# jnvance/DMRG.x

Hardware: AMD Instinct MI355X
Metric: superblock MatMults/sec inside the ground-state eigensolve (Lanczos step = 1 MatMult + reorthogonalisation) (higher is better)
Workload: dtype f64

## Files before the change

dmrg.x_amd/csrc/eigs.hip:

```cpp
#include "krylov.h"
#include <mutex>
#include <algorithm>
#include <chrono>
#include <cmath>
#include <cstring>
#include <cstddef>

namespace dmrgx {
namespace {

constexpr int DOT_BLOCKS = 1024, DOT_THREADS = 256, DOT_CHUNK = 8, MAX_NCV = 64, FUSE_NV = 24, GD_NV = 8;

template <bool VEC2>
__global__ void __launch_bounds__(DOT_THREADS)
multi_dot_kernel(const double* __restrict__ V, int64_t ldv, int nv, const double* __restrict__ w, int64_t n, double* __restrict__ partial)
{
    __shared__ double red[DOT_THREADS / 64][DOT_CHUNK];
    const int v0 = blockIdx.y * DOT_CHUNK;
    double acc[DOT_CHUNK];
#pragma unroll
    for (int i = 0; i < DOT_CHUNK; ++i) acc[i] = 0.0;
    if (VEC2) {
        const double2* __restrict__ w2 = reinterpret_cast<const double2*>(w);
        for (int64_t e = (int64_t)blockIdx.x * DOT_THREADS + threadIdx.x; e < n / 2; e += (int64_t)gridDim.x * DOT_THREADS) {
            const double2 wv = w2[e];
#pragma unroll
            for (int i = 0; i < DOT_CHUNK; ++i) {
                const int v = v0 + i;
                if (v < nv) { const double2 x = reinterpret_cast<const double2*>(V + (int64_t)v * ldv)[e]; acc[i] += x.x * wv.x + x.y * wv.y; }
                else if (v == nv) acc[i] += wv.x * wv.x + wv.y * wv.y;
            }
        }
    } else {
        for (int64_t e = (int64_t)blockIdx.x * DOT_THREADS + threadIdx.x; e < n; e += (int64_t)gridDim.x * DOT_THREADS) {
            const double wv = w[e];
#pragma unroll
            for (int i = 0; i < DOT_CHUNK; ++i) {
                const int v = v0 + i;
                if (v < nv) acc[i] += V[(int64_t)v * ldv + e] * wv;
                else if (v == nv) acc[i] += wv * wv;
            }
        }
    }
    const int lane = threadIdx.x & 63, wave = threadIdx.x >> 6;
#pragma unroll
    for (int i = 0; i < DOT_CHUNK; ++i) {
        const double s = wave_sum(acc[i]);
        if (lane == 0) red[wave][i] = s;
    }
    __syncthreads();
    if (threadIdx.x < DOT_CHUNK) {
        double s = 0.0;
        for (int wv = 0; wv < DOT_THREADS / 64; ++wv) s += red[wv][threadIdx.x];
        partial[(int64_t)(v0 + threadIdx.x) * gridDim.x + blockIdx.x] = s;
    }
}

__global__ void __launch_bounds__(DOT_THREADS)
reduce_partials_kernel(const double* __restrict__ partial, double* __restrict__ out, int count, int nblk)
{
    const int i = blockIdx.x;
    if (i >= count) return;
    const double s = sum_partials<DOT_THREADS>(partial + (int64_t)i * nblk, nblk);
    if (threadIdx.x == 0) out[i] = s;
}

__global__ void __launch_bounds__(DOT_THREADS)
multi_axpy_kernel(const double* __restrict__ V, int64_t ldv, int nv, const double* __restrict__ c, double* __restrict__ w, int64_t n,
                  double* __restrict__ partial, double* __restrict__ hacc)
{
    __shared__ double cs[MAX_NCV + 1];
    if (threadIdx.x < nv) cs[threadIdx.x] = c[threadIdx.x];
    __syncthreads();
    if (blockIdx.x == 0 && threadIdx.x < nv && hacc) hacc[threadIdx.x] += cs[threadIdx.x];
    double nrm = 0.0;
    for (int64_t e = (int64_t)blockIdx.x * DOT_THREADS + threadIdx.x; e < n; e += (int64_t)gridDim.x * DOT_THREADS) {
        double x = w[e];
        for (int i = 0; i < nv; ++i) x -= cs[i] * V[(int64_t)i * ldv + e];
        w[e] = x;
        nrm += x * x;
    }
    nrm = block_sum<DOT_THREADS>(nrm);
    if (threadIdx.x == 0) partial[blockIdx.x] = nrm;
}

template <int NVMAX>
__global__ void __launch_bounds__(DOT_THREADS)
axpy_dot_kernel(const double* __restrict__ V, int64_t ldv, int nv, const double* __restrict__ c, double* __restrict__ w, int64_t n,
                double* __restrict__ partial, double* __restrict__ hacc)
{
    __shared__ double cs[NVMAX];
    __shared__ double red[DOT_THREADS / 64][NVMAX + 1];
    if (threadIdx.x < nv) cs[threadIdx.x] = c[threadIdx.x];
    __syncthreads();
    if (blockIdx.x == 0 && threadIdx.x < nv && hacc) hacc[threadIdx.x] += cs[threadIdx.x];
    double acc[NVMAX + 1];
#pragma unroll
    for (int i = 0; i <= NVMAX; ++i) acc[i] = 0.0;
    for (int64_t e = (int64_t)blockIdx.x * DOT_THREADS + threadIdx.x; e < n; e += (int64_t)gridDim.x * DOT_THREADS) {
        double v[NVMAX];
#pragma unroll
        for (int i = 0; i < NVMAX; ++i) v[i] = i < nv ? V[(int64_t)i * ldv + e] : 0.0;
        double x = w[e];
#pragma unroll
        for (int i = 0; i < NVMAX; ++i) if (i < nv) x -= cs[i] * v[i];
        w[e] = x;
#pragma unroll
        for (int i = 0; i < NVMAX; ++i) if (i < nv) acc[i] += v[i] * x;
        acc[NVMAX] += x * x;
    }
    const int lane = threadIdx.x & 63, wave = threadIdx.x >> 6;
#pragma unroll
    for (int i = 0; i <= NVMAX; ++i) {
        if (i < nv || i == NVMAX) {
            const double s2 = wave_sum(acc[i]);
            if (lane == 0) red[wave][i] = s2;
        }
    }
    __syncthreads();
    if (threadIdx.x <= nv) {
        const int src = threadIdx.x < nv ? threadIdx.x : NVMAX;
        double s2 = 0.0;
        for (int wv = 0; wv < DOT_THREADS / 64; ++wv) s2 += red[wv][src];
        partial[(int64_t)threadIdx.x * gridDim.x + blockIdx.x] = s2;
    }
}

template <bool VEC2>
__global__ void __launch_bounds__(DOT_THREADS)
axpy_normalise_kernel(const double* __restrict__ V, int64_t ldv, int nv, const double* __restrict__ c, const double* __restrict__ w,
                      double* __restrict__ dst, int64_t n, double* __restrict__ beta2_out, double* __restrict__ hacc)
{
    __shared__ double cs[MAX_NCV + 2];
    if (threadIdx.x <= nv) cs[threadIdx.x] = c[threadIdx.x];
    __syncthreads();
    if (blockIdx.x == 0 && threadIdx.x < nv && hacc) hacc[threadIdx.x] += cs[threadIdx.x];
    double s2 = cs[nv], sc = 0.0;
    for (int i = 0; i < nv; ++i) { s2 -= cs[i] * cs[i]; sc += cs[i] * cs[i]; }
    s2 = s2 > 0.0 ? s2 : 0.0;
    if (blockIdx.x == 0 && threadIdx.x == 0 && beta2_out) *beta2_out = s2;
    const double inv = s2 > 1e-290 ? 1.0 / sqrt(s2) : 0.0;
    if (sc <= 1e-27 * cs[nv]) nv = 0;
    if (VEC2) {
        const double2* __restrict__ w2 = reinterpret_cast<const double2*>(w);
        double2* __restrict__ d2 = reinterpret_cast<double2*>(dst);
        for (int64_t e = (int64_t)blockIdx.x * DOT_THREADS + threadIdx.x; e < n / 2; e += (int64_t)gridDim.x * DOT_THREADS) {
            double2 x = w2[e];
            for (int i = 0; i < nv; ++i) { const double2 v = reinterpret_cast<const double2*>(V + (int64_t)i * ldv)[e]; x.x -= cs[i] * v.x; x.y -= cs[i] * v.y; }
            x.x *= inv; x.y *= inv;
            d2[e] = x;
        }
    } else {
        for (int64_t e = (int64_t)blockIdx.x * DOT_THREADS + threadIdx.x; e < n; e += (int64_t)gridDim.x * DOT_THREADS) {
            double x = w[e];
            for (int i = 0; i < nv; ++i) x -= cs[i] * V[(int64_t)i * ldv + e];
            dst[e] = x * inv;
        }
    }
}

__global__ void norm_after_projection_kernel(const double* __restrict__ c, int nv, double* __restrict__ nrm2)
{
    if (threadIdx.x == 0 && blockIdx.x == 0) { double s = c[nv]; for (int i = 0; i < nv; ++i) s -= c[i] * c[i]; *nrm2 = s > 0.0 ? s : 0.0; }
}

__global__ void scale_copy_kernel(const double* __restrict__ src, double* __restrict__ dst, int64_t n, const double* __restrict__ nrm2)
{
    const double s2 = *nrm2;
    const double inv = s2 > 1e-290 ? 1.0 / sqrt(s2) : 0.0;
    for (int64_t e = (int64_t)blockIdx.x * blockDim.x + threadIdx.x; e < n; e += (int64_t)gridDim.x * blockDim.x) dst[e] = src[e] * inv;
}

__global__ void __launch_bounds__(DOT_THREADS)
basis_rotate_kernel(const double* __restrict__ V, int64_t ldv, int m, const double* __restrict__ Q, int ldq, int k,
                    double* __restrict__ out, int64_t ldo, int64_t n)
{
    __shared__ double qs[MAX_NCV * DOT_CHUNK];
    const int j0 = blockIdx.y * DOT_CHUNK;
    for (int t = threadIdx.x; t < m * DOT_CHUNK; t += DOT_THREADS) {
        const int i = t / DOT_CHUNK, j = t % DOT_CHUNK;
        qs[t] = (j0 + j < k) ? Q[i * ldq + j0 + j] : 0.0;
    }
    __syncthreads();
    for (int64_t e = (int64_t)blockIdx.x * DOT_THREADS + threadIdx.x; e < n; e += (int64_t)gridDim.x * DOT_THREADS) {
        double acc[DOT_CHUNK];
#pragma unroll
        for (int j = 0; j < DOT_CHUNK; ++j) acc[j] = 0.0;
        for (int i = 0; i < m; ++i) {
            const double v = V[(int64_t)i * ldv + e];
#pragma unroll
            for (int j = 0; j < DOT_CHUNK; ++j) acc[j] += v * qs[i * DOT_CHUNK + j];
        }
#pragma unroll
        for (int j = 0; j < DOT_CHUNK; ++j) if (j0 + j < k) out[(int64_t)(j0 + j) * ldo + e] = acc[j];
    }
}

constexpr int GD_MAX = FUSE_NV;
constexpr int GD_LD = GD_MAX;
struct GdState {
    double G[GD_MAX * GD_LD];
    double Y[GD_MAX * GD_LD];
    double th[GD_MAX];
    double y[GD_MAX];
    double yprev[GD_MAX];
    double Q[GD_MAX * GD_LD];
    double theta;
    double hv0_2;
    double e0[GD_MAX];
    int after_restart;
    int pad_;
};

constexpr int RITZ_THREADS = 64;
__global__ void __launch_bounds__(RITZ_THREADS)
gd_ritz_kernel(GdState* __restrict__ S, const double* __restrict__ col_src, int col_is_partial, int nblk, int mm, int warm, int restart, int keep)
{
    __shared__ double A[GD_MAX][GD_MAX + 1], Qa[GD_MAX][GD_MAX + 1], Yn[GD_MAX][GD_MAX + 1], Yp[GD_MAX][GD_MAX + 1];
    __shared__ double col[GD_MAX + 1], cs_c[GD_MAX / 2], cs_s[GD_MAX / 2], dg[GD_MAX], thp[GD_MAX], ths[GD_MAX];
    __shared__ int pp[GD_MAX / 2], qq[GD_MAX / 2], perm[GD_MAX];
    __shared__ double offn, dgn;
    const int tid = threadIdx.x, lane = tid;
    const int j = mm - 1;
    if (warm && mm > 1) {
        for (int e = tid; e < (mm - 1) * (mm - 1); e += RITZ_THREADS) Yp[e / (mm - 1)][e % (mm - 1)] = S->Y[(e / (mm - 1)) * GD_LD + e % (mm - 1)];
        if (tid < mm - 1) thp[tid] = S->th[tid];
    }
    const double yold = tid < GD_MAX ? S->y[tid] : 0.0;
    const int was_restart = S->after_restart;
    if (col_is_partial) {
        constexpr int PER = DOT_BLOCKS / RITZ_THREADS;
        for (int i0 = 0; i0 <= mm; i0 += 4) {
            double t[4][PER];
#pragma unroll
            for (int g = 0; g < 4; ++g)
#pragma unroll
                for (int u = 0; u < PER; ++u) t[g][u] = (i0 + g <= mm && tid + u * RITZ_THREADS < nblk) ? col_src[(int64_t)(i0 + g) * nblk + tid + u * RITZ_THREADS] : 0.0;
#pragma unroll
            for (int g = 0; g < 4; ++g) {
                double v = 0.0;
#pragma unroll
                for (int u = 0; u < PER; ++u) v += t[g][u];
                v = wave_sum(v);
                if (lane == 0 && i0 + g <= mm) col[i0 + g] = v;
            }
        }
    } else if (tid <= mm) col[tid] = col_src[tid];
    __syncthreads();
    if (tid < mm) { S->G[tid * GD_LD + j] = col[tid]; S->G[j * GD_LD + tid] = col[tid]; }
    if (tid == 0 && mm == 1) S->hv0_2 = col[1];
    if (tid < GD_MAX && mm == 1) S->e0[tid] = tid == 0 ? 1.0 : 0.0;
    if (tid < mm) S->yprev[tid] = was_restart ? (tid == 0 ? 1.0 : 0.0) : (tid < mm - 1 ? yold : 0.0);
    if (tid == 0) S->after_restart = restart;
    const int n = (mm + 1) & ~1;
    const int mp = mm - 1;
    for (int e = tid; e < n * n; e += RITZ_THREADS) {
        const int a = e / n, b = e % n;
        double v = 0.0;
        if (a < mm && b < mm) {
            if (!warm || mp == 0) v = (a == j || b == j) ? col[a == j ? b : a] : S->G[a * GD_LD + b];
            else if (a < mp && b < mp) v = a == b ? thp[a] : 0.0;
            else if (a == mp && b == mp) v = col[j];
            else {
                const int i = a == mp ? b : a;
                for (int k = 0; k < mp; ++k) v += Yp[k][i] * col[k];
            }
        }
        A[a][b] = v;
        Qa[a][b] = a == b ? 1.0 : 0.0;
    }
    __syncthreads();
    constexpr int UMAX = (GD_MAX / 2 * GD_MAX + RITZ_THREADS - 1) / RITZ_THREADS;
    int wk[UMAX], wi[UMAX];
#pragma unroll
    for (int u = 0; u < UMAX; ++u) { const int e = tid + u * RITZ_THREADS; wk[u] = e < (n / 2) * n ? e / n : -1; wi[u] = e % n; }
    for (int sweep = 0; sweep < 30 && n > 1; ++sweep) {
        {
            double off = 0.0, dgs = 0.0;
#pragma unroll
            for (int u = 0; u < UMAX; ++u) {
                if (wk[u] < 0) continue;
                const double v0 = A[wk[u]][wi[u]], v1 = A[wk[u] + n / 2][wi[u]];
                if (wk[u] == wi[u]) dgs += v0 * v0; else off += v0 * v0;
                if (wk[u] + n / 2 == wi[u]) dgs += v1 * v1; else off += v1 * v1;
            }
            off = wave_sum(off); dgs = wave_sum(dgs);
            if (lane == 0) { offn = off; dgn = dgs; }
        }
        __syncthreads();
        if (offn <= 1e-29 * (dgn + offn) || offn == 0.0) break;
        for (int r = 0; r < n - 1; ++r) {
            if (tid < n / 2) {
                const int k = tid;
                int p0 = r + k, q0 = r - k + (n - 1);
                if (p0 >= n - 1) p0 -= n - 1;
                if (q0 >= n - 1) q0 -= n - 1;
                if (k == 0) { p0 = r; q0 = n - 1; }
                const int p = min(p0, q0), q = max(p0, q0);
                const double apq = A[p][q];
                double c = 1.0, sn = 0.0;
                if (apq != 0.0) {
                    const double th = 0.5 * (A[q][q] - A[p][p]);
                    const double h = sqrt(th * th + apq * apq);
                    const double t = apq / (th + (th >= 0.0 ? h : -h));
                    c = rsqrt(1.0 + t * t); sn = t * c;
                }
                pp[k] = p; qq[k] = q; cs_c[k] = c; cs_s[k] = sn;
            }
            __syncthreads();
#pragma unroll
            for (int u = 0; u < UMAX; ++u) {
                if (wk[u] < 0) continue;
                const int k = wk[u], i = wi[u];
                const int p = pp[k], q = qq[k];
                const double c = cs_c[k], sn = cs_s[k];
                const double aip = A[i][p], aiq = A[i][q];
                A[i][p] = c * aip - sn * aiq; A[i][q] = sn * aip + c * aiq;
                const double qip = Qa[i][p], qiq = Qa[i][q];
                Qa[i][p] = c * qip - sn * qiq; Qa[i][q] = sn * qip + c * qiq;
            }
            __syncthreads();
#pragma unroll
            for (int u = 0; u < UMAX; ++u) {
                if (wk[u] < 0) continue;
                const int k = wk[u], i = wi[u];
                const int p = pp[k], q = qq[k];
                const double c = cs_c[k], sn = cs_s[k];
                const double api = A[p][i], aqi = A[q][i];
                A[p][i] = i == q ? 0.0 : c * api - sn * aqi; A[q][i] = i == p ? 0.0 : sn * api + c * aqi;
            }
            __syncthreads();
        }
    }
    if (tid < mm) dg[tid] = A[tid][tid];
    __syncthreads();
    if (tid < mm) {
        int rank = 0;
        for (int o = 0; o < mm; ++o) rank += (dg[o] < dg[tid] || (dg[o] == dg[tid] && o < tid)) ? 1 : 0;
        perm[rank] = tid;
    }
    __syncthreads();
    for (int e = tid; e < mm * mm; e += RITZ_THREADS) {
        const int i = e / mm, cidx = e % mm;
        const int src = perm[cidx];
        double v;
        if (!warm || mp == 0 || i == mp) v = Qa[i][src];
        else { v = 0.0; for (int k = 0; k < mp; ++k) v += Yp[i][k] * Qa[k][src]; }
        Yn[i][cidx] = v;
    }
    __syncthreads();
    for (int e = tid; e < mm * mm; e += RITZ_THREADS) S->Y[(e / mm) * GD_LD + (e % mm)] = Yn[e / mm][e % mm];
    if (tid < mm) { ths[tid] = dg[perm[tid]]; S->th[tid] = ths[tid]; S->y[tid] = Yn[tid][0]; }
    if (tid == 0) S->theta = dg[perm[0]];
    if (!restart) return;
    __syncthreads();
    const int kk = keep + 1;
    {
        double pv = lane < mm ? S->yprev[lane] : 0.0;
        for (int pass = 0; pass < 2; ++pass)
            for (int c = 0; c < keep; ++c) {
                const double qc = lane < mm ? Yn[lane][c] : 0.0;
                double d = qc * pv;
#pragma unroll
                for (int o = 32; o > 0; o >>= 1) d += __shfl_xor(d, o, 64);
                pv -= d * qc;
            }
        double nn = pv * pv;
#pragma unroll
        for (int o = 32; o > 0; o >>= 1) nn += __shfl_xor(nn, o, 64);
        const double last = nn > 1e-16 ? pv / sqrt(nn) : (lane < mm ? Yn[lane][keep] : 0.0);
        if (lane < mm) A[lane][keep] = last;
    }
    for (int e = tid; e < mm * keep; e += RITZ_THREADS) A[e / keep][e % keep] = Yn[e / keep][e % keep];
    __syncthreads();
    for (int e = tid; e < mm * kk; e += RITZ_THREADS) S->Q[e] = A[e / kk][e % kk];
    for (int e = tid; e < mm * mm; e += RITZ_THREADS) Qa[e / mm][e % mm] = S->G[(e / mm) * GD_LD + e % mm];
    __syncthreads();
    if (tid < mm) { double v = 0.0; for (int b = 0; b < mm; ++b) v += Qa[tid][b] * A[b][keep]; col[tid] = v; }
    __syncthreads();
    if (tid < kk) { double v = 0.0; for (int a = 0; a < mm; ++a) v += A[a][tid] * col[a]; dg[tid] = v; }
    __syncthreads();
    for (int e = tid; e < GD_MAX * GD_LD; e += RITZ_THREADS) {
        const int a = e / GD_LD, b = e % GD_LD;
        double v = 0.0;
        if (a < keep && b < keep) v = a == b ? ths[a] : 0.0;
        else if (a < kk && b < kk) v = dg[a == keep ? b : a];
        S->G[e] = v;
    }
}

template <int NVMAX, bool DOTS>
__global__ void __launch_bounds__(DOT_THREADS)
ritz_precond_kernel(const double* __restrict__ V, const double* __restrict__ W, int64_t ldv, int nv, const GdState* __restrict__ S,
                    const double* __restrict__ D, double floor_rel, double* __restrict__ t, int64_t n, double* __restrict__ partial)
{
    __shared__ double ys[NVMAX];
    __shared__ double red[DOT_THREADS / 64][NVMAX + 2];
    if (threadIdx.x < NVMAX) ys[threadIdx.x] = threadIdx.x < nv ? S->y[threadIdx.x] : 0.0;
    const double theta = S->theta;
    const double floor_ = floor_rel * fmax(1.0, fabs(theta)) * 1e-2 + 1e-12;
    __syncthreads();
    double acc[NVMAX + 2];
#pragma unroll
    for (int i = 0; i < NVMAX + 2; ++i) acc[i] = 0.0;
    const double2* __restrict__ D2 = reinterpret_cast<const double2*>(D);
    double2* __restrict__ t2 = reinterpret_cast<double2*>(t);
    for (int64_t e = (int64_t)blockIdx.x * DOT_THREADS + threadIdx.x; e < n / 2; e += (int64_t)gridDim.x * DOT_THREADS) {
        double2 v[NVMAX];
        double2 u = {0.0, 0.0}, hu = {0.0, 0.0};
#pragma unroll
        for (int i = 0; i < NVMAX; ++i)
            if (i < nv) {
                v[i] = reinterpret_cast<const double2*>(V + (int64_t)i * ldv)[e];
                const double2 w = reinterpret_cast<const double2*>(W + (int64_t)i * ldv)[e];
                u.x += ys[i] * v[i].x; u.y += ys[i] * v[i].y; hu.x += ys[i] * w.x; hu.y += ys[i] * w.y;
            } else v[i] = double2{0.0, 0.0};
        const double2 r = {hu.x - theta * u.x, hu.y - theta * u.y};
        const double2 dv = D2[e];
        double2 den = {theta - dv.x, theta - dv.y};
        if (fabs(den.x) < floor_) den.x = den.x < 0.0 ? -floor_ : floor_;
        if (fabs(den.y) < floor_) den.y = den.y < 0.0 ? -floor_ : floor_;
        const double2 te = {r.x / den.x, r.y / den.y};
        t2[e] = te;
        if (DOTS) {
#pragma unroll
            for (int i = 0; i < NVMAX; ++i) if (i < nv) acc[i] += v[i].x * te.x + v[i].y * te.y;
            acc[NVMAX] += te.x * te.x + te.y * te.y;
        }
        acc[NVMAX + 1] += r.x * r.x + r.y * r.y;
    }
    const int lane = threadIdx.x & 63, wave = threadIdx.x >> 6;
#pragma unroll
    for (int i = 0; i < NVMAX + 2; ++i) {
        if ((DOTS && (i < nv || i == NVMAX)) || i == NVMAX + 1) {
            const double s2 = wave_sum(acc[i]);
            if (lane == 0) red[wave][i] = s2;
        }
    }
    __syncthreads();
    if (DOTS) {
        if (threadIdx.x <= nv + 1) {
            const int src = threadIdx.x < nv ? threadIdx.x : (threadIdx.x == nv ? NVMAX : NVMAX + 1);
            double s2 = 0.0;
            for (int wv = 0; wv < DOT_THREADS / 64; ++wv) s2 += red[wv][src];
            partial[(int64_t)threadIdx.x * gridDim.x + blockIdx.x] = s2;
        }
    } else if (threadIdx.x == 0) {
        double s2 = 0.0;
        for (int wv = 0; wv < DOT_THREADS / 64; ++wv) s2 += red[wv][NVMAX + 1];
        partial[blockIdx.x] = s2;
    }
}

__global__ void gd_zero_pads_kernel(double* __restrict__ W, int64_t ld, int count, int64_t n, double* __restrict__ t, double* __restrict__ D)
{
    for (int j = threadIdx.x; j < count; j += blockDim.x) W[(int64_t)j * ld + n] = 0.0;
    if (threadIdx.x == 0) { t[n] = 0.0; D[n] = 0.0; }
}

__global__ void __launch_bounds__(DOT_THREADS)
gd_reduce_look_kernel(const double* __restrict__ partial, double* __restrict__ out, int count, int nblk, int look_idx, int look_only,
                      const GdState* __restrict__ S, double* __restrict__ look)
{
    const int i = blockIdx.x;
    if (i >= count) return;
    double t = 0.0;
    if (!look_only) {
        t = sum_partials<DOT_THREADS>(partial + (int64_t)i * nblk, nblk);
        if (threadIdx.x == 0) out[i] = t;
    } else if (threadIdx.x == 0) t = out[i];
    if (threadIdx.x == 0 && i == look_idx) { look[0] = t; look[1] = S->theta; look[2] = S->hv0_2; }
}

__global__ void random_fill_kernel(double* __restrict__ v, int64_t n, uint64_t seed, int64_t index_offset)
{
    for (int64_t e = (int64_t)blockIdx.x * blockDim.x + threadIdx.x; e < n; e += (int64_t)gridDim.x * blockDim.x) {
        uint64_t z = seed + 0x9E3779B97F4A7C15ull * (uint64_t)(e + index_offset + 1);
        z = (z ^ (z >> 30)) * 0xBF58476D1CE4E5B9ull;
        z = (z ^ (z >> 27)) * 0x94D049BB133111EBull;
        z ^= z >> 31;
        v[e] = (double)(z >> 11) * (2.0 / 9007199254740992.0) - 1.0;
    }
}

void jacobi_eigh(int n, std::vector<double>& A, std::vector<double>& w, std::vector<double>& Q)
{
    Q.assign((size_t)n * n, 0.0);
    for (int i = 0; i < n; ++i) Q[(size_t)i * n + i] = 1.0;
    for (int sweep = 0; sweep < 60; ++sweep) {
        double off = 0.0, diag = 0.0;
        for (int i = 0; i < n; ++i) { diag += A[(size_t)i * n + i] * A[(size_t)i * n + i]; for (int j = i + 1; j < n; ++j) off += A[(size_t)i * n + j] * A[(size_t)i * n + j]; }
        if (off <= 1e-32 * (diag + off) || off == 0.0) break;
        for (int p = 0; p < n - 1; ++p)
            for (int q = p + 1; q < n; ++q) {
                const double apq = A[(size_t)p * n + q];
                if (apq == 0.0) continue;
                const double app = A[(size_t)p * n + p], aqq = A[(size_t)q * n + q];
                const double tau = (aqq - app) / (2.0 * apq);
                const double t = (tau >= 0 ? 1.0 : -1.0) / (std::fabs(tau) + std::sqrt(1.0 + tau * tau));
                const double c = 1.0 / std::sqrt(1.0 + t * t), s = t * c;
                for (int k = 0; k < n; ++k) {
                    const double akp = A[(size_t)k * n + p], akq = A[(size_t)k * n + q];
                    A[(size_t)k * n + p] = c * akp - s * akq; A[(size_t)k * n + q] = s * akp + c * akq;
                }
                for (int k = 0; k < n; ++k) {
                    const double apk = A[(size_t)p * n + k], aqk = A[(size_t)q * n + k];
                    A[(size_t)p * n + k] = c * apk - s * aqk; A[(size_t)q * n + k] = s * apk + c * aqk;
                }
                for (int k = 0; k < n; ++k) {
                    const double qkp = Q[(size_t)k * n + p], qkq = Q[(size_t)k * n + q];
                    Q[(size_t)k * n + p] = c * qkp - s * qkq; Q[(size_t)k * n + q] = s * qkp + c * qkq;
                }
            }
    }
    std::vector<int> idx(n);
    for (int i = 0; i < n; ++i) idx[i] = i;
    std::sort(idx.begin(), idx.end(), [&](int a, int b) { return A[(size_t)a * n + a] < A[(size_t)b * n + b]; });
    w.resize(n);
    std::vector<double> Qs((size_t)n * n);
    for (int j = 0; j < n; ++j) { w[j] = A[(size_t)idx[j] * n + idx[j]]; for (int i = 0; i < n; ++i) Qs[(size_t)i * n + j] = Q[(size_t)i * n + idx[j]]; }
    Q.swap(Qs);
}

}
}

using namespace dmrgx;

namespace {
std::mutex g_ct_mutex;
double g_ct_allgather_ms = 0.0, g_ct_apply_ms = 0.0;
int64_t g_ct_matvecs = 0;
struct CommTimer {
    hipStream_t st;
    std::vector<hipEvent_t> ev;
    size_t used = 0;
    explicit CommTimer(hipStream_t s) : st(s) {}
    void mark()
    {
        if (used == ev.size()) { hipEvent_t e; if (hipEventCreate(&e) != hipSuccess) return; ev.push_back(e); }
        (void)hipEventRecord(ev[used++], st);
    }
    ~CommTimer()
    {
        double ag = 0.0, ap = 0.0; int64_t nmv = 0;
        for (size_t i = 0; i + 2 < used; i += 3) {
            float a = 0.f, b = 0.f;
            if (hipEventSynchronize(ev[i + 2]) != hipSuccess) break;
            if (hipEventElapsedTime(&a, ev[i], ev[i + 1]) == hipSuccess && hipEventElapsedTime(&b, ev[i + 1], ev[i + 2]) == hipSuccess) { ag += a; ap += b; ++nmv; }
        }
        for (hipEvent_t e : ev) (void)hipEventDestroy(e);
        if (nmv) { std::lock_guard<std::mutex> lk(g_ct_mutex); g_ct_allgather_ms += ag; g_ct_apply_ms += ap; g_ct_matvecs += nmv; }
    }
};
}

extern "C" dmrgx_status dmrgx_eigs_comm_timing(double* allgather_ms, double* apply_ms, int64_t* n_matvec, int32_t reset)
{
    std::lock_guard<std::mutex> lk(g_ct_mutex);
    if (allgather_ms) *allgather_ms = g_ct_allgather_ms;
    if (apply_ms) *apply_ms = g_ct_apply_ms;
    if (n_matvec) *n_matvec = g_ct_matvecs;
    if (reset) { g_ct_allgather_ms = 0.0; g_ct_apply_ms = 0.0; g_ct_matvecs = 0; }
    return DMRGX_OK;
}

namespace {

bool eigs_trace()
{
    static const bool on = getenv("DMRGX_EIGS_TRACE") != nullptr;
    return on;
}

constexpr size_t LOOK_STRIDE = (size_t)(MAX_NCV + 1) * (MAX_NCV + 2);
struct HostLooks {
    double* pin = nullptr;
    hipEvent_t ev[3] = {nullptr, nullptr, nullptr};
    double* start_norm2() const { return pin; }
    double* gd_look() const { return pin + 1; }
    double* lanczos_look(int slot) const { return pin + 4 + (size_t)slot * LOOK_STRIDE; }
};
dmrgx_status host_looks(HostLooks** out)
{
    static thread_local HostLooks h;
    if (!h.pin) {
        for (hipEvent_t& e : h.ev) if (!e) DMRGX_HIP(hipEventCreateWithFlags(&e, hipEventDisableTiming));
        DMRGX_HIP(hipHostMalloc((void**)&h.pin, (4 + 2 * LOOK_STRIDE) * sizeof(double), hipHostMallocDefault));
    }
    *out = &h;
    return DMRGX_OK;
}

struct EigsRun {
    dmrgx_kron_plan* const plan;
    const dmrgx_eigs_opts* const opts;
    double* const e0;
    double* const psi_full;
    dmrgx_eigs_stats* const stats;
    const hipStream_t st;
    dmrgx_kron_info I;
    int64_t n = 0, N = 0;
    bool dist = false, hooks = false;
    std::chrono::steady_clock::time_point t_begin;
    HostLooks* host = nullptr;
    CommTimer ctimer;
    DevBuf dX, dPartial, dV, dW, dTmp, dScal;
    DevBuf dQ;
    DevBuf dT, dD, dState, dLook;
    int64_t ld = 0;
    double* V = nullptr;
    double *c1 = nullptr, *c2 = nullptr, *nrm = nullptr;

    EigsRun(dmrgx_kron_plan* p, const dmrgx_eigs_opts* o, double* e, double* psi, dmrgx_eigs_stats* s, hipStream_t stream)
        : plan(p), opts(o), e0(e), psi_full(psi), stats(s), st(stream), ctimer(stream) {}

    dmrgx_status init()
    {
        DMRGX_CHK(dmrgx_kron_plan_info(plan, &I));
        dist = I.vec_len != I.n_states;
        hooks = opts->allgather && opts->allreduce_sum;
        if (dist && !hooks && !opts->comm) DMRGX_FAIL(DMRGX_ERR_ARG, "eigs_lowest: a striped plan needs a communicator (opts->comm) or the allgather/allreduce hooks");
        n = I.local_len; N = I.n_states;
        t_begin = std::chrono::steady_clock::now();
        return host_looks(&host);
    }
    double seconds() const { return std::chrono::duration<double>(std::chrono::steady_clock::now() - t_begin).count(); }
    double* psi_local() const { return dist ? psi_full + I.local_offset : psi_full; }

    dmrgx_status alloc_shared()
    {
        if (dist) DMRGX_CHK(dX.alloc_f64((size_t)I.vec_len, st));
        return dPartial.alloc_f64((size_t)(MAX_NCV + DOT_CHUNK + 2) * DOT_BLOCKS, st);
    }
    void layout(double* scratch) { V = dV.as<double>(); c1 = scratch; c2 = c1 + (MAX_NCV + 2); nrm = c2 + (MAX_NCV + 2); }
    void release_work() { for (DevBuf* b : {&dX, &dPartial, &dV, &dW, &dTmp, &dScal, &dQ, &dT, &dD, &dState, &dLook}) b->release(); }

    dmrgx_status allreduce(double* buf, int64_t count)
    {
        if (!dist) return DMRGX_OK;
        return hooks ? opts->allreduce_sum(opts->user, buf, count, st) : dmrgx_comm_allreduce_sum(opts->comm, buf, count, st);
    }
    dmrgx_status gather_full(double* full)
    {
        return hooks ? opts->allgather(opts->user, full, I.seg_stride, st) : dmrgx_comm_allgather(opts->comm, full, I.seg_stride, st);
    }
    dmrgx_status matvec(const double* v_local, double* y_local)
    {
        if (!dist) return dmrgx_kron_apply(plan, v_local, y_local, st);
        DMRGX_HIP(hipMemcpyAsync(dX.as<double>() + I.local_offset, v_local, (size_t)n * sizeof(double), hipMemcpyDeviceToDevice, st));
        ctimer.mark();
        DMRGX_CHK(gather_full(dX.as<double>()));
        ctimer.mark();
        const dmrgx_status rc = dmrgx_kron_apply(plan, dX.as<double>(), y_local, st);
        ctimer.mark();
        return rc;
    }
    dmrgx_status start_vector(double* dst)
    {
        if (opts->use_initial) { DMRGX_HIP(hipMemcpyAsync(dst, psi_full + I.local_offset, (size_t)n * sizeof(double), hipMemcpyDeviceToDevice, st)); return DMRGX_OK; }
        if (!dist) { hipLaunchKernelGGL(random_fill_kernel, dim3(1024), dim3(256), 0, st, dst, n, opts->seed, (int64_t)0); DMRGX_HIP(hipGetLastError()); return DMRGX_OK; }
        DevBuf ref;
        DMRGX_CHK(ref.alloc((size_t)N * sizeof(double)));
        hipLaunchKernelGGL(random_fill_kernel, dim3(1024), dim3(256), 0, st, ref.as<double>(), N, opts->seed, (int64_t)0);
        DMRGX_HIP(hipGetLastError());
        DMRGX_CHK(dmrgx_kron_vec_to_striped(plan, ref.as<double>(), dX.as<double>(), st));
        DMRGX_HIP(hipMemcpyAsync(dst, dX.as<double>() + I.local_offset, (size_t)n * sizeof(double), hipMemcpyDeviceToDevice, st));
        DMRGX_HIP(hipStreamSynchronize(st));
        return DMRGX_OK;
    }
    dmrgx_status fetch_start_norm2(const double* dev)
    {
        if (!opts->use_initial) return DMRGX_OK;
        *host->start_norm2() = 0.0;
        DMRGX_HIP(hipMemcpyAsync(host->start_norm2(), dev, sizeof(double), hipMemcpyDeviceToHost, st));
        return DMRGX_OK;
    }
    bool start_too_light() const { return opts->use_initial && opts->min_initial_norm2 > 0.0 && !(*host->start_norm2() >= opts->min_initial_norm2); }

    dmrgx_status multi_dot(int nv, const double* x, double* out, bool reduce)
    {
        const int chunks = (nv + 1 + DOT_CHUNK - 1) / DOT_CHUNK;
        if (ld % 2 == 0) hipLaunchKernelGGL(multi_dot_kernel<true>, dim3(DOT_BLOCKS, chunks), dim3(DOT_THREADS), 0, st, V, ld, nv, x, ld, dPartial.as<double>());
        else hipLaunchKernelGGL(multi_dot_kernel<false>, dim3(DOT_BLOCKS, chunks), dim3(DOT_THREADS), 0, st, V, ld, nv, x, ld, dPartial.as<double>());
        DMRGX_HIP(hipGetLastError());
        if (!reduce) return DMRGX_OK;
        hipLaunchKernelGGL(reduce_partials_kernel, dim3(nv + 1), dim3(DOT_THREADS), 0, st, dPartial.as<double>(), out, nv + 1, DOT_BLOCKS);
        DMRGX_HIP(hipGetLastError());
        return allreduce(out, nv + 1);
    }
    template <int NV> dmrgx_status project_and_dot(int nv, double* x, double* hacc)
    {
        hipLaunchKernelGGL(axpy_dot_kernel<NV>, dim3(DOT_BLOCKS), dim3(DOT_THREADS), 0, st, V, ld, nv, c1, x, ld, dPartial.as<double>(), hacc);
        DMRGX_HIP(hipGetLastError());
        hipLaunchKernelGGL(reduce_partials_kernel, dim3(nv + 1), dim3(DOT_THREADS), 0, st, dPartial.as<double>(), c2, nv + 1, DOT_BLOCKS);
        DMRGX_HIP(hipGetLastError());
        return allreduce(c2, nv + 1);
    }
    dmrgx_status project_and_normalise(int nv, const double* x, double* dst, double* beta2, double* hacc)
    {
        if (ld % 2 == 0) hipLaunchKernelGGL(axpy_normalise_kernel<true>, dim3(DOT_BLOCKS), dim3(DOT_THREADS), 0, st, V, ld, nv, c2, x, dst, ld, beta2, hacc);
        else hipLaunchKernelGGL(axpy_normalise_kernel<false>, dim3(DOT_BLOCKS), dim3(DOT_THREADS), 0, st, V, ld, nv, c2, x, dst, ld, beta2, hacc);
        DMRGX_HIP(hipGetLastError());
        return DMRGX_OK;
    }
    dmrgx_status finish_vector(const double* src)
    {
        DMRGX_CHK(multi_dot(0, src, c1, true));
        DMRGX_HIP(hipMemcpyAsync(nrm, c1, sizeof(double), hipMemcpyDeviceToDevice, st));
        hipLaunchKernelGGL(scale_copy_kernel, dim3(1024), dim3(256), 0, st, src, psi_local(), n, (const double*)nrm);
        DMRGX_HIP(hipGetLastError());
        if (dist) DMRGX_CHK(gather_full(psi_full));
        DMRGX_HIP(hipStreamSynchronize(st));
        return DMRGX_OK;
    }
    void finish(double lambda, double resid, int n_matvec, int restarts, int converged)
    {
        *e0 = lambda;
        if (!stats) return;
        stats->n_matvec = n_matvec; stats->n_restart = restarts; stats->converged = converged; stats->start_rejected = 0; stats->residual = resid;
        stats->seconds = seconds();
    }
    dmrgx_status solve_again(const dmrgx_eigs_opts& o2, int n_matvec, int restarts, bool rejected)
    {
        release_work();
        dmrgx_eigs_stats s2;
        memset(&s2, 0, sizeof(s2));
        const dmrgx_status rc = dmrgx_eigs_lowest(plan, &o2, e0, psi_full, &s2, (void*)st);
        if (stats) {
            *stats = s2; stats->n_matvec += n_matvec; stats->n_restart += restarts; stats->seconds = seconds();
            if (rejected) stats->start_rejected = 1;
        }
        return rc;
    }
    dmrgx_status eigs_lanczos();
    dmrgx_status eigs_davidson();
};

struct Ritz {
    std::vector<double> th, Q;
    double resid;
};
Ritz ritz_of_leading(int mm, int m, int row, const std::vector<double>& hbuf, const std::vector<double>& kept)
{
    const int k = (int)kept.size();
    std::vector<double> A((size_t)mm * mm, 0.0);
    for (int j = 0; j < mm; ++j) for (int i = 0; i <= j; ++i) {
        const double v = j >= k ? hbuf[(size_t)j * row + i] : (i == j ? kept[j] : 0.0);
        A[(size_t)i * mm + j] = v; A[(size_t)j * mm + i] = v;
    }
    Ritz r;
    jacobi_eigh(mm, A, r.th, r.Q);
    r.resid = std::fabs(std::sqrt(std::max(0.0, hbuf[(size_t)(mm - 1) * row + m + 1])) * r.Q[(size_t)(mm - 1) * mm + 0]);
    return r;
}

dmrgx_status EigsRun::eigs_lanczos()
{
    int m = opts->ncv > 0 ? opts->ncv : 16;
    m = (int)std::min<int64_t>(std::min(m, MAX_NCV), N);
    m = (int)std::max<int64_t>(m, std::min<int64_t>(2, N));
    if (m < 1) DMRGX_FAIL(DMRGX_ERR_ARG, "eigs_lowest: empty problem");
    const int max_it = opts->max_it > 0 ? opts->max_it : std::max<int>(100, (int)(2 * N / m));
    const double tol = opts->tol > 0 ? opts->tol : 1e-8;

    ld = n;
    DMRGX_CHK(dV.alloc_f64((size_t)(m + 1) * n, st));
    DMRGX_CHK(dW.alloc_f64((size_t)n, st));
    DMRGX_CHK(dTmp.alloc_f64((size_t)(m / 2 + 2) * n, st));
    DMRGX_CHK(alloc_shared());
    const int row = m + 2;
    DMRGX_CHK(dScal.alloc_f64((size_t)((m + 1) * row + 3 * (MAX_NCV + 2)), st));
    DMRGX_CHK(dQ.alloc_f64((size_t)MAX_NCV * MAX_NCV, st));
    layout(dScal.as<double>() + (size_t)(m + 1) * row);
    double* const w = dW.as<double>();
    auto Hrow = [&](int j) { return dScal.as<double>() + (size_t)j * row; };
    auto vec = [&](int j) { return V + (size_t)j * n; };
    DMRGX_HIP(zero_async(dV.p, dV.bytes, st));
    DMRGX_HIP(zero_async(dW.p, dW.bytes, st));
    if (dist) DMRGX_HIP(zero_async(dX.p, dX.bytes, st));

    DMRGX_CHK(start_vector(w));
    DMRGX_CHK(multi_dot(0, w, c1, true));
    DMRGX_CHK(fetch_start_norm2(c1));
    DMRGX_HIP(hipMemcpyAsync(nrm, c1, sizeof(double), hipMemcpyDeviceToDevice, st));
    hipLaunchKernelGGL(scale_copy_kernel, dim3(1024), dim3(256), 0, st, w, vec(0), n, nrm);
    DMRGX_HIP(hipGetLastError());

    const bool looks = opts->max_matvec <= 0;
    int look_mm[2] = {0, 0};
    std::vector<double> kept, y((size_t)m, 0.0), hbuf((size_t)(m + 1) * row), Qdev;
    int k = 0, n_matvec = 0, restarts = 0, converged = 0;
    double resid = 0.0, lambda = 0.0;
    auto null_start = [&]() { return opts->use_initial && restarts == 0 && k == 0 && ((!(std::fabs(hbuf[0]) > 0.0) && !(hbuf[(size_t)m + 1] > 0.0)) || start_too_light()); };
    auto redo_from_random = [&]() -> dmrgx_status {
        dmrgx_eigs_opts o2 = *opts;
        o2.use_initial = 0;
        return solve_again(o2, n_matvec, 0, true);
    };
    while (true) {
        DMRGX_HIP(zero_async(Hrow(k), (size_t)(m + 1 - k) * row * sizeof(double), st));
        int jend = m;
        if (opts->max_matvec > 0) jend = std::min(m, k + std::max(0, opts->max_matvec - n_matvec));
        const bool capped = jend < m || (opts->max_matvec > 0 && n_matvec + (m - k) >= opts->max_matvec);
        bool early = false;
        for (int j = k; j < jend; ++j) {
            DMRGX_CHK(matvec(vec(j), w));
            ++n_matvec;
            const int nv = j + 1;
            DMRGX_CHK(multi_dot(nv, w, c1, true));
            if (nv <= FUSE_NV) DMRGX_CHK(project_and_dot<FUSE_NV>(nv, w, Hrow(j)));
            else {
                hipLaunchKernelGGL(multi_axpy_kernel, dim3(DOT_BLOCKS), dim3(DOT_THREADS), 0, st, V, n, nv, c1, w, n, dPartial.as<double>(), Hrow(j));
                DMRGX_HIP(hipGetLastError());
                DMRGX_CHK(multi_dot(nv, w, c1, true));
                DMRGX_HIP(hipMemcpyAsync(c2, c1, (size_t)(nv + 1) * sizeof(double), hipMemcpyDeviceToDevice, st));
            }
            DMRGX_CHK(project_and_normalise(nv, w, vec(j + 1), Hrow(j) + m + 1, Hrow(j)));
            if (looks && j + 1 < m) {
                const int slot = j & 1;
                DMRGX_HIP(hipMemcpyAsync(host->lanczos_look(slot), dScal.p, (size_t)(m + 1) * row * sizeof(double), hipMemcpyDeviceToHost, st));
                DMRGX_HIP(hipEventRecord(host->ev[slot], st));
                look_mm[slot] = j + 1;
            }
            if (looks && j > k && look_mm[(j - 1) & 1] == j) {
                const int slot = (j - 1) & 1;
                look_mm[slot] = 0;
                DMRGX_HIP(hipEventSynchronize(host->ev[slot]));
                std::copy(host->lanczos_look(slot), host->lanczos_look(slot) + (size_t)(m + 1) * row, hbuf.begin());
                if (null_start()) { DMRGX_HIP(hipStreamSynchronize(st)); return redo_from_random(); }
                const Ritz look = ritz_of_leading(j, m, row, hbuf, kept);
                if (eigs_trace()) fprintf(stderr, "[eigs] look at matvec %d (queued: %d): theta %.12f  |r| %.3e  (target %.3e)\n", n_matvec - 1, n_matvec, look.th[0], look.resid, tol * std::fabs(look.th[0]));
                if (look.resid <= tol * std::max(std::fabs(look.th[0]), 1e-300)) { jend = j + 1; early = true; break; }
            }
        }
        look_mm[0] = look_mm[1] = 0;
        DMRGX_HIP(hipMemcpyAsync(hbuf.data(), dScal.p, (size_t)(m + 1) * row * sizeof(double), hipMemcpyDeviceToHost, st));
        DMRGX_HIP(hipStreamSynchronize(st));
        if (null_start()) return redo_from_random();
        const int mm = jend;
        if (mm < 1) break;
        const Ritz ritz = ritz_of_leading(mm, m, row, hbuf, kept);
        lambda = ritz.th[0];
        resid = ritz.resid;
        std::fill(y.begin(), y.end(), 0.0);
        for (int i = 0; i < mm; ++i) y[i] = ritz.Q[(size_t)i * mm + 0];
        ++restarts;
        if (mm < m) { if (early) converged = 1; break; }
        if (resid <= tol * std::max(std::fabs(lambda), 1e-300) || m == N) { converged = 1; break; }
        if (restarts >= max_it || capped) break;
        const int kk = std::max(1, std::min(m / 2, m - 1));
        Qdev.assign((size_t)m * kk, 0.0);
        for (int i = 0; i < m; ++i) for (int j = 0; j < kk; ++j) Qdev[(size_t)i * kk + j] = ritz.Q[(size_t)i * m + j];
        DMRGX_HIP(h2d_async(dQ.p, Qdev.data(), Qdev.size() * sizeof(double), st));
        hipLaunchKernelGGL(basis_rotate_kernel, dim3(1024, (kk + DOT_CHUNK - 1) / DOT_CHUNK), dim3(DOT_THREADS), 0, st,
                           V, n, m, dQ.as<double>(), kk, kk, dTmp.as<double>(), n, n);
        DMRGX_HIP(hipGetLastError());
        DMRGX_HIP(hipMemcpyAsync(V, dTmp.p, (size_t)kk * n * sizeof(double), hipMemcpyDeviceToDevice, st));
        DMRGX_HIP(hipMemcpyAsync(vec(kk), vec(m), (size_t)n * sizeof(double), hipMemcpyDeviceToDevice, st));
        DMRGX_HIP(hipStreamSynchronize(st));
        kept.assign(ritz.th.begin(), ritz.th.begin() + kk);
        k = kk;
    }
    DMRGX_HIP(h2d_async(dQ.p, y.data(), y.size() * sizeof(double), st));
    hipLaunchKernelGGL(basis_rotate_kernel, dim3(1024, 1), dim3(DOT_THREADS), 0, st, V, n, m, dQ.as<double>(), 1, 1, w, n, n);
    DMRGX_HIP(hipGetLastError());
    DMRGX_CHK(finish_vector(w));
    finish(lambda, resid, n_matvec, restarts, converged);
    if (!converged) DMRGX_FAIL(DMRGX_ERR_NOTCONV, "eigs_lowest: not converged after %d restarts (residual %.3e)", restarts, resid);
    return DMRGX_OK;
}

dmrgx_status EigsRun::eigs_davidson()
{
    ld = (n + 1) & ~(int64_t)1;
    int m = opts->ncv > 0 ? opts->ncv : GD_NV;
    m = (int)std::min<int64_t>(std::min(m, GD_MAX - 1), N);
    if (m < 2) DMRGX_FAIL(DMRGX_ERR_ARG, "eigs_lowest (gd): needs at least a two-dimensional search space");
    if (m < 3 && N >= 3) m = 3;
    const int keep = std::max(1, std::min(opts->gd_minv > 0 ? opts->gd_minv : 1, m - 2));
    const int kk = keep + 1;
    const int max_mv = opts->max_it > 0 ? opts->max_it * 16 : std::max<int>(1600, (int)(2 * N));
    const int hand_over = 96;
    const double tol = opts->tol > 0 ? opts->tol : 1e-8;
    const int nblk = DOT_BLOCKS;
    const bool fused = m <= GD_NV;

    auto mark = [&](const char* what) {
        if (!eigs_trace()) return;
        (void)hipStreamSynchronize(st);
        fprintf(stderr, "[eigs gd] setup %-12s t = %.3f ms\n", what, 1e3 * seconds());
    };
    mark("enter");
    DMRGX_CHK(dV.alloc_f64((size_t)(m + 1) * ld, st));
    DMRGX_CHK(dW.alloc_f64((size_t)(m + 1) * ld, st));
    DMRGX_CHK(dT.alloc_f64((size_t)ld, st));
    DMRGX_CHK(dD.alloc_f64((size_t)ld, st));
    DMRGX_CHK(dTmp.alloc_f64((size_t)kk * ld, st));
    DMRGX_CHK(alloc_shared());
    DMRGX_CHK(dScal.alloc_f64((size_t)(3 * (MAX_NCV + 2)), st));
    DMRGX_CHK(dState.alloc(sizeof(GdState)));
    layout(dScal.as<double>());
    double* const W = dW.as<double>();
    double* const t = dT.as<double>();
    double* const partial = dPartial.as<double>();
    const double* const D = dD.as<double>();
    const GdState* const S = dState.as<GdState>();
    const double* const S_y = (const double*)((const char*)S + offsetof(GdState, y));
    const double* const S_e0 = (const double*)((const char*)S + offsetof(GdState, e0));
    const double* const S_Q = (const double*)((const char*)S + offsetof(GdState, Q));
    auto vec = [&](int j) { return V + (size_t)j * ld; };
    auto wvec = [&](int j) { return W + (size_t)j * ld; };
    if (dist) { DMRGX_HIP(zero_async(dV.p, dV.bytes, st)); DMRGX_HIP(zero_async(dW.p, dW.bytes, st)); }
    if (dist) DMRGX_HIP(zero_async(dT.p, dT.bytes, st));
    DMRGX_HIP(zero_async(dState.p, dState.bytes, st));
    if (dist) DMRGX_HIP(zero_async(dX.p, dX.bytes, st));
    mark("buffers");
    DMRGX_CHK(dmrgx_kron_diag(plan, dD.as<double>(), st));
    if (ld != n) {
        hipLaunchKernelGGL(gd_zero_pads_kernel, dim3(1), dim3(64), 0, st, W, ld, m + 1, n, t, dD.as<double>());
        DMRGX_HIP(hipGetLastError());
    }
    mark("diagonal");
    auto orthonormalise_tail = [&](int nv, double* x, double* dst) -> dmrgx_status {
        DMRGX_CHK(nv <= GD_NV ? project_and_dot<GD_NV>(nv, x, nullptr) : project_and_dot<FUSE_NV>(nv, x, nullptr));
        return project_and_normalise(nv, x, dst, nullptr, nullptr);
    };

    DMRGX_CHK(start_vector(t));
    DMRGX_CHK(multi_dot(0, t, c1, true));
    DMRGX_CHK(orthonormalise_tail(0, t, vec(0)));
    DMRGX_CHK(fetch_start_norm2(c2));
    mark("start vector");

    double* const h_look = host->gd_look();
    const hipEvent_t ev_look = host->ev[2];
    DMRGX_CHK(dLook.alloc(4 * sizeof(double)));
    double* const look = dLook.as<double>();
    int j = 0, n_matvec = 0, restarts = 0, converged = 0;
    double lambda = 0.0, resid = 0.0;
    const double floor_rel = 1e-3;
    bool warm = false;
    bool rotated = false;
    int mm = 0;
    dmrgx_eigs_opts o2 = *opts;
    o2.method = 0;
    while (true) {
        DMRGX_CHK(matvec(vec(j), wvec(j)));
        ++n_matvec;
        mm = j + 1;
        const bool restart = mm == m;
        DMRGX_CHK(multi_dot(mm, wvec(j), c1, dist));
        hipLaunchKernelGGL(gd_ritz_kernel, dim3(1), dim3(RITZ_THREADS), 0, st, dState.as<GdState>(), dist ? (const double*)c1 : (const double*)partial, dist ? 0 : 1, nblk, mm, warm ? 1 : 0, restart ? 1 : 0, keep);
        DMRGX_HIP(hipGetLastError());
        warm = !restart;
        rotated = false;
        const int look_idx = fused ? mm + 1 : 0;
        double* red_out = fused ? c1 : nrm;
        if (fused) hipLaunchKernelGGL((ritz_precond_kernel<GD_NV, true>), dim3(nblk), dim3(DOT_THREADS), 0, st, (const double*)V, (const double*)W, ld, mm, S, D, floor_rel, t, ld, partial);
        else hipLaunchKernelGGL((ritz_precond_kernel<FUSE_NV, false>), dim3(nblk), dim3(DOT_THREADS), 0, st, (const double*)V, (const double*)W, ld, mm, S, D, floor_rel, t, ld, partial);
        DMRGX_HIP(hipGetLastError());
        const int nred = fused ? mm + 2 : 1;
        hipLaunchKernelGGL(gd_reduce_look_kernel, dim3(nred), dim3(DOT_THREADS), 0, st, (const double*)partial, red_out, nred, nblk, look_idx, 0, S, look);
        DMRGX_HIP(hipGetLastError());
        if (dist) {
            DMRGX_CHK(allreduce(red_out, nred));
            hipLaunchKernelGGL(gd_reduce_look_kernel, dim3(nred), dim3(DOT_THREADS), 0, st, (const double*)partial, red_out, nred, nblk, look_idx, 1, S, look);
            DMRGX_HIP(hipGetLastError());
        }
        DMRGX_HIP(hipMemcpyAsync(h_look, look, 3 * sizeof(double), hipMemcpyDeviceToHost, st));
        DMRGX_HIP(hipEventRecord(ev_look, st));
        const bool may_continue = mm < N && n_matvec < max_mv && n_matvec < hand_over;
        if (may_continue) {
            bool have_dots = fused;
            if (restart) {
                for (double* B : {V, W}) {
                    hipLaunchKernelGGL(basis_rotate_kernel, dim3(1024, (kk + DOT_CHUNK - 1) / DOT_CHUNK), dim3(DOT_THREADS), 0, st, (const double*)B, ld, m, S_Q, kk, kk,
                                       dTmp.as<double>(), ld, ld);
                    DMRGX_HIP(hipGetLastError());
                    DMRGX_HIP(hipMemcpyAsync(B, dTmp.p, (size_t)kk * ld * sizeof(double), hipMemcpyDeviceToDevice, st));
                }
                j = kk - 1;
                ++restarts;
                rotated = true;
                have_dots = false;
            }
            if (!have_dots) DMRGX_CHK(multi_dot(j + 1, t, c1, true));
            DMRGX_CHK(orthonormalise_tail(j + 1, t, vec(j + 1)));
        }
        DMRGX_HIP(hipEventSynchronize(ev_look));
        resid = std::sqrt(std::max(h_look[0], 0.0));
        lambda = h_look[1];
        if (n_matvec == 1 && (!(h_look[2] > 0.0) || start_too_light())) {
            DMRGX_HIP(hipStreamSynchronize(st));
            o2.use_initial = 0;
            return solve_again(o2, n_matvec, 0, true);
        }
        if (eigs_trace()) fprintf(stderr, "[eigs gd] matvec %d: basis %d theta %.12f  |r| %.3e  (target %.3e)  t = %.3f ms\n", n_matvec, mm, lambda, resid, tol * std::fabs(lambda), 1e3 * seconds());
        if (resid <= tol * std::max(std::fabs(lambda), 1e-300) || mm == N) { converged = 1; break; }
        if (n_matvec >= max_mv) break;
        if (n_matvec >= hand_over) {
            hipLaunchKernelGGL(basis_rotate_kernel, dim3(1024, 1), dim3(DOT_THREADS), 0, st, (const double*)V, ld, mm, S_y, 1, 1, psi_local(), n, n);
            DMRGX_HIP(hipGetLastError());
            DMRGX_HIP(hipStreamSynchronize(st));
            o2.use_initial = 1; o2.min_initial_norm2 = 0.0;
            return solve_again(o2, n_matvec, restarts, false);
        }
        ++j;
    }
    hipLaunchKernelGGL(basis_rotate_kernel, dim3(1024, 1), dim3(DOT_THREADS), 0, st, (const double*)V, ld, rotated ? 1 : mm, rotated ? S_e0 : S_y, 1, 1, t, ld, ld);
    DMRGX_HIP(hipGetLastError());
    DMRGX_CHK(finish_vector(t));
    finish(lambda, resid, n_matvec, restarts, converged);
    if (eigs_trace()) fprintf(stderr, "[eigs gd] done: %d MatMults, %.3f ms\n", n_matvec, 1e3 * seconds());
    if (!converged) DMRGX_FAIL(DMRGX_ERR_NOTCONV, "eigs_lowest (gd): not converged after %d MatMults (residual %.3e)", n_matvec, resid);
    return DMRGX_OK;
}

}

extern "C" dmrgx_status dmrgx_eigs_lowest(dmrgx_kron_plan* plan, const dmrgx_eigs_opts* opts, double* e0,
                                          double* psi_full, dmrgx_eigs_stats* stats, void* stream)
{
    if (!plan || !opts || !e0 || !psi_full) DMRGX_FAIL(DMRGX_ERR_ARG, "eigs_lowest: null argument");
    EigsRun R(plan, opts, e0, psi_full, stats, (hipStream_t)stream);
    DMRGX_CHK(R.init());
    const bool gd_space = std::min<int64_t>(opts->ncv > 0 ? opts->ncv : 16, R.N) >= 2;
    if (opts->method == 1 && opts->use_initial && opts->max_matvec <= 0 && gd_space) return R.eigs_davidson();
    return R.eigs_lanczos();
}
```

Before: 380.7.

## Fuse Lanczos thick restart into an in-place basis rotation kernel

Replaces the restart sequence (rotate the basis into a temporary buffer, copy it back, then copy the residual vector) with a single kernel. Each thread reads all m basis rows for its element pair, computes kk rotated outputs in registers and writes them back into V in place, along with the residual vector. It also drops the temp allocation and the up-front zeroing of V. The final Ritz vector rotation now uses only the rows actually filled. This removes the extra device-to-device traffic and launches per restart, at the cost of high register pressure for large kk and correctness depending on per-thread in-place ordering.

```diff
diff --git a/dmrg.x_amd/csrc/eigs.hip b/dmrg.x_amd/csrc/eigs.hip
--- a/dmrg.x_amd/csrc/eigs.hip
+++ b/dmrg.x_amd/csrc/eigs.hip
@@ -193,6 +193,40 @@
         }
 #pragma unroll
         for (int j = 0; j < DOT_CHUNK; ++j) if (j0 + j < k) out[(int64_t)(j0 + j) * ldo + e] = acc[j];
+    }
+}
+
+template <int KMAX, bool VEC>
+__global__ void __launch_bounds__(DOT_THREADS)
+basis_restart_kernel(double* V, int64_t ldv, int m, const double* __restrict__ Q, int ldq, int kk, int64_t n)
+{
+    __shared__ double qs[MAX_NCV * KMAX];
+    for (int t = threadIdx.x; t < m * KMAX; t += DOT_THREADS) {
+        const int i = t / KMAX, j = t % KMAX;
+        qs[t] = j < kk ? Q[i * ldq + j] : 0.0;
+    }
+    __syncthreads();
+    constexpr int ROWS = 8;
+    for (int64_t p = (int64_t)blockIdx.x * DOT_THREADS + threadIdx.x; 2 * p < n; p += (int64_t)gridDim.x * DOT_THREADS) {
+        const int64_t e = 2 * p;
+        double2 acc[KMAX];
+#pragma unroll
+        for (int j = 0; j < KMAX; ++j) acc[j] = double2{0.0, 0.0};
+        for (int i0 = 0; i0 < m; i0 += ROWS) {
+            double2 v[ROWS];
+#pragma unroll
+            for (int u = 0; u < ROWS; ++u) v[u] = i0 + u < m ? load2<VEC>(V + (int64_t)(i0 + u) * ldv, e, n) : double2{0.0, 0.0};
+#pragma unroll
+            for (int u = 0; u < ROWS; ++u) {
+                if (i0 + u >= m) break;
+#pragma unroll
+                for (int j = 0; j < KMAX; ++j) { const double q = qs[(i0 + u) * KMAX + j]; acc[j].x += v[u].x * q; acc[j].y += v[u].y * q; }
+            }
+        }
+        const double2 r = load2<VEC>(V + (int64_t)m * ldv, e, n);
+#pragma unroll
+        for (int j = 0; j < KMAX; ++j) if (j < kk) store2<VEC>(V + (int64_t)j * ldv, e, n, acc[j]);
+        store2<VEC>(V + (int64_t)kk * ldv, e, n, r);
     }
 }
 
@@ -592,6 +626,30 @@
     return DMRGX_OK;
 }
 
+bool eigs_old_restart()
+{
+    const char* s = getenv("DMRGX_EIGS_OLD");
+    return s && (atoi(s) & 1);
+}
+
+dmrgx_status launch_basis_restart(double* V, int64_t ld, int m, const double* Q, int kk, int64_t n, hipStream_t st)
+{
+    if (m < 2 || m > MAX_NCV || kk < 1 || kk >= m || kk > 32) DMRGX_FAIL(DMRGX_ERR_ARG, "basis_restart: m = %d, kk = %d", m, kk);
+    const dim3 grid(1024), block(DOT_THREADS);
+    const bool vec = ld % 2 == 0 && (uintptr_t)V % 16 == 0;
+#define DMRGX_RESTART(KMAX)                                                                                               \
+    do {                                                                                                                  \
+        if (vec) hipLaunchKernelGGL((basis_restart_kernel<KMAX, true>), grid, block, 0, st, V, ld, m, Q, kk, kk, n);      \
+        else hipLaunchKernelGGL((basis_restart_kernel<KMAX, false>), grid, block, 0, st, V, ld, m, Q, kk, kk, n);         \
+    } while (0)
+    if (kk <= 8) DMRGX_RESTART(8);
+    else if (kk <= 16) DMRGX_RESTART(16);
+    else DMRGX_RESTART(32);
+#undef DMRGX_RESTART
+    DMRGX_HIP(hipGetLastError());
+    return DMRGX_OK;
+}
+
 struct EigsRun {
     dmrgx_kron_plan* const plan;
     const dmrgx_eigs_opts* const opts;
@@ -767,7 +825,8 @@
     ld = n;
     DMRGX_CHK(dV.alloc_f64((size_t)(m + 1) * n, st));
     DMRGX_CHK(dW.alloc_f64((size_t)n, st));
-    DMRGX_CHK(dTmp.alloc_f64((size_t)(m / 2 + 2) * n, st));
+    const bool old_restart = eigs_old_restart();
+    if (old_restart) DMRGX_CHK(dTmp.alloc_f64((size_t)(m / 2 + 2) * n, st));
     DMRGX_CHK(alloc_shared());
     const int row = m + 2;
     DMRGX_CHK(dScal.alloc_f64((size_t)((m + 1) * row + 3 * (MAX_NCV + 2)), st));
@@ -776,7 +835,7 @@
     double* const w = dW.as<double>();
     auto Hrow = [&](int j) { return dScal.as<double>() + (size_t)j * row; };
     auto vec = [&](int j) { return V + (size_t)j * n; };
-    DMRGX_HIP(zero_async(dV.p, dV.bytes, st));
+    if (old_restart) DMRGX_HIP(zero_async(dV.p, dV.bytes, st));
     DMRGX_HIP(zero_async(dW.p, dW.bytes, st));
     if (dist) DMRGX_HIP(zero_async(dX.p, dX.bytes, st));
 
@@ -790,7 +849,7 @@
     const bool looks = opts->max_matvec <= 0;
     int look_mm[2] = {0, 0};
     std::vector<double> kept, y((size_t)m, 0.0), hbuf((size_t)(m + 1) * row), Qdev;
-    int k = 0, n_matvec = 0, restarts = 0, converged = 0;
+    int k = 0, n_matvec = 0, restarts = 0, converged = 0, ritz_rows = 0;
     double resid = 0.0, lambda = 0.0;
     auto null_start = [&]() { return opts->use_initial && restarts == 0 && k == 0 && ((!(std::fabs(hbuf[0]) > 0.0) && !(hbuf[(size_t)m + 1] > 0.0)) || start_too_light()); };
     auto redo_from_random = [&]() -> dmrgx_status {
@@ -845,6 +904,7 @@
         resid = ritz.resid;
         std::fill(y.begin(), y.end(), 0.0);
         for (int i = 0; i < mm; ++i) y[i] = ritz.Q[(size_t)i * mm + 0];
+        ritz_rows = mm;
         ++restarts;
         if (mm < m) { if (early) converged = 1; break; }
         if (resid <= tol * std::max(std::fabs(lambda), 1e-300) || m == N) { converged = 1; break; }
@@ -853,17 +913,20 @@
         Qdev.assign((size_t)m * kk, 0.0);
         for (int i = 0; i < m; ++i) for (int j = 0; j < kk; ++j) Qdev[(size_t)i * kk + j] = ritz.Q[(size_t)i * m + j];
         DMRGX_HIP(h2d_async(dQ.p, Qdev.data(), Qdev.size() * sizeof(double), st));
-        hipLaunchKernelGGL(basis_rotate_kernel, dim3(1024, (kk + DOT_CHUNK - 1) / DOT_CHUNK), dim3(DOT_THREADS), 0, st,
-                           V, n, m, dQ.as<double>(), kk, kk, dTmp.as<double>(), n, n);
-        DMRGX_HIP(hipGetLastError());
-        DMRGX_HIP(hipMemcpyAsync(V, dTmp.p, (size_t)kk * n * sizeof(double), hipMemcpyDeviceToDevice, st));
-        DMRGX_HIP(hipMemcpyAsync(vec(kk), vec(m), (size_t)n * sizeof(double), hipMemcpyDeviceToDevice, st));
+        if (!old_restart) DMRGX_CHK(launch_basis_restart(V, n, m, dQ.as<double>(), kk, n, st));
+        else {
+            hipLaunchKernelGGL(basis_rotate_kernel, dim3(1024, (kk + DOT_CHUNK - 1) / DOT_CHUNK), dim3(DOT_THREADS), 0, st,
+                               V, n, m, dQ.as<double>(), kk, kk, dTmp.as<double>(), n, n);
+            DMRGX_HIP(hipGetLastError());
+            DMRGX_HIP(hipMemcpyAsync(V, dTmp.p, (size_t)kk * n * sizeof(double), hipMemcpyDeviceToDevice, st));
+            DMRGX_HIP(hipMemcpyAsync(vec(kk), vec(m), (size_t)n * sizeof(double), hipMemcpyDeviceToDevice, st));
+        }
         DMRGX_HIP(hipStreamSynchronize(st));
         kept.assign(ritz.th.begin(), ritz.th.begin() + kk);
         k = kk;
     }
     DMRGX_HIP(h2d_async(dQ.p, y.data(), y.size() * sizeof(double), st));
-    hipLaunchKernelGGL(basis_rotate_kernel, dim3(1024, 1), dim3(DOT_THREADS), 0, st, V, n, m, dQ.as<double>(), 1, 1, w, n, n);
+    hipLaunchKernelGGL(basis_rotate_kernel, dim3(1024, 1), dim3(DOT_THREADS), 0, st, V, n, old_restart ? m : ritz_rows, dQ.as<double>(), 1, 1, w, n, n);
     DMRGX_HIP(hipGetLastError());
     DMRGX_CHK(finish_vector(w));
     finish(lambda, resid, n_matvec, restarts, converged);
@@ -1029,3 +1092,21 @@
     if (opts->method == 1 && opts->use_initial && opts->max_matvec <= 0 && gd_space) return R.eigs_davidson();
     return R.eigs_lanczos();
 }
+
+extern "C" dmrgx_status dmrgx_debug_eigs_restart(double* V, int64_t ld, int32_t m, const double* Q_dev, int32_t kk, int64_t n, int32_t old_form, void* stream)
+{
+    const hipStream_t st = (hipStream_t)stream;
+    if (!V || !Q_dev || n < 1 || ld < n || m < 2 || m > MAX_NCV || kk < 1 || kk >= m) DMRGX_FAIL(DMRGX_ERR_ARG, "debug_eigs_restart: bad argument");
+    if (!old_form) DMRGX_CHK(launch_basis_restart(V, ld, m, Q_dev, kk, n, st));
+    else {
+        DevBuf tmp;
+        DMRGX_CHK(tmp.alloc_f64((size_t)kk * n, st));
+        hipLaunchKernelGGL(basis_rotate_kernel, dim3(1024, (kk + DOT_CHUNK - 1) / DOT_CHUNK), dim3(DOT_THREADS), 0, st, (const double*)V, ld, m, Q_dev, kk, kk, tmp.as<double>(), n, n);
+        DMRGX_HIP(hipGetLastError());
+        DMRGX_HIP(hipMemcpy2DAsync(V, (size_t)ld * sizeof(double), tmp.p, (size_t)n * sizeof(double), (size_t)n * sizeof(double), (size_t)kk, hipMemcpyDeviceToDevice, st));
+        DMRGX_HIP(hipMemcpyAsync(V + (size_t)kk * ld, V + (size_t)m * ld, (size_t)n * sizeof(double), hipMemcpyDeviceToDevice, st));
+        DMRGX_HIP(hipStreamSynchronize(st));
+    }
+    DMRGX_HIP(hipStreamSynchronize(st));
+    return DMRGX_OK;
+}
```

Measured after the change: 383.6, median of 6. About the same (+0.7%).
